# arpg/vicalib

Hardware: AMD Instinct MI355X
Metric: corner_residuals_per_sec (higher is better)
Workload: dtype f64

## Files before the change

vicalib_amd/csrc/vc_imu.hpp:

```cpp
#pragma once
#include "vc_math.hpp"

namespace vc {

struct D1 { double a, v; };
VC_HD D1 mk(double a, double v = 0.0) { D1 r; r.a = a; r.v = v; return r; }
VC_HD D1 operator+(D1 x, D1 y) { return mk(x.a + y.a, x.v + y.v); }
VC_HD D1 operator-(D1 x, D1 y) { return mk(x.a - y.a, x.v - y.v); }
VC_HD D1 operator-(D1 x) { return mk(-x.a, -x.v); }
VC_HD D1 operator*(D1 x, D1 y) { return mk(x.a * y.a, x.a * y.v + x.v * y.a); }
VC_HD D1 operator/(D1 x, D1 y) { const double inv = fast_rcp(y.a), q = x.a * inv; return mk(q, (x.v - q * y.v) * inv); }
VC_HD D1 operator+(D1 x, double s) { return mk(x.a + s, x.v); }
VC_HD D1 operator+(double s, D1 x) { return mk(x.a + s, x.v); }
VC_HD D1 operator-(D1 x, double s) { return mk(x.a - s, x.v); }
VC_HD D1 operator-(double s, D1 x) { return mk(s - x.a, -x.v); }
VC_HD D1 operator*(D1 x, double s) { return mk(x.a * s, x.v * s); }
VC_HD D1 operator*(double s, D1 x) { return mk(x.a * s, x.v * s); }
VC_HD D1 operator/(D1 x, double s) { const double inv = 1.0 / s; return mk(x.a * inv, x.v * inv); }
VC_HD D1 operator/(double s, D1 y) { const double inv = fast_rcp(y.a); return mk(s * inv, -s * inv * inv * y.v); }
VC_HD bool operator<(D1 x, double y) { return x.a < y; }
VC_HD bool operator>(D1 x, double y) { return x.a > y; }
VC_HD D1 sqrt(D1 x) { double s, is; fast_sqrt_rsqrt(x.a, &s, &is); return mk(s, 0.5 * x.v * is); }
VC_HD D1 sin(D1 x) { return mk(::sin(x.a), ::cos(x.a) * x.v); }
VC_HD D1 cos(D1 x) { return mk(::cos(x.a), -::sin(x.a) * x.v); }
// ... 304 lines not shown
  J[0 * 6 + 3] = 0.5 * q0; J[0 * 6 + 4] = -0.5 * q3; J[0 * 6 + 5] = 0.5 * q2;
  J[1 * 6 + 3] = 0.5 * q3; J[1 * 6 + 4] = 0.5 * q0; J[1 * 6 + 5] = -0.5 * q1;
  J[2 * 6 + 3] = -0.5 * q2; J[2 * 6 + 4] = 0.5 * q1; J[2 * 6 + 5] = 0.5 * q0;
  J[3 * 6 + 3] = -0.5 * q1; J[3 * 6 + 4] = -0.5 * q2; J[3 * 6 + 5] = -0.5 * q3;
  J[4 * 6 + 0] = 1.0 - 2.0 * (q2 * q2 + q3 * q3); J[4 * 6 + 1] = 2.0 * (q1 * q2 - q0 * q3); J[4 * 6 + 2] = 2.0 * (q1 * q3 + q0 * q2);
  J[5 * 6 + 0] = 2.0 * (q1 * q2 + q0 * q3); J[5 * 6 + 1] = 1.0 - 2.0 * (q1 * q1 + q3 * q3); J[5 * 6 + 2] = 2.0 * (q2 * q3 - q0 * q1);
  J[6 * 6 + 0] = 2.0 * (q1 * q3 - q0 * q2); J[6 * 6 + 1] = 2.0 * (q2 * q3 + q0 * q1); J[6 * 6 + 2] = 1.0 - 2.0 * (q1 * q1 + q2 * q2);
}

VC_HD void imu_block_direction(const ImuView& buf, double t_start, double t_end, const double* w_sqrt, int rotation_only,
                               const double* T2, const double* T1, const double* v2, const double* v1, const double* gdir,
                               const double* b, const double* sf, double toff, int dir, double* r, double* dr) {
  D1 P[35];
  for (int i = 0; i < 7; ++i) { P[i] = mk(T2[i]); P[7 + i] = mk(T1[i]); }
  for (int i = 0; i < 3; ++i) { P[14 + i] = mk(v2[i]); P[17 + i] = mk(v1[i]); }
  P[20] = mk(gdir[0]); P[21] = mk(gdir[1]);
  for (int i = 0; i < 6; ++i) { P[22 + i] = mk(b[i]); P[28 + i] = mk(sf[i]); }
  P[34] = mk(toff);
  for (int i = 0; i < 35; ++i) P[i].v = (i == dir) ? 1.0 : 0.0;
  D1 res[9];
  imu_residual<D1>(buf, t_start, t_end, w_sqrt, rotation_only, P, P + 7, P + 14, P + 17, P + 20, P + 22, P + 28, P[34], res);
  for (int i = 0; i < 9; ++i) { r[i] = res[i].a; dr[i] = res[i].v; }
}

constexpr int kDeltaCols = 14;

template <class T> struct DeltaAcc { T q[4], p[3], v[3], t; };
template <class T> VC_HD void imu_delta_append(DeltaAcc<T>* A, const PoseV<T>& d, T dt) {
  T rp[3], rv[3], q[4];
  tq_rotate(A->q, d.p, rp);
  tq_rotate(A->q, d.v, rv);
  tq_mul(A->q, d.q, q);
  for (int i = 0; i < 3; ++i) {
    A->p[i] = (A->p[i] + A->v[i] * dt) + rp[i];
    A->v[i] = A->v[i] + rv[i];
  }
  for (int i = 0; i < 4; ++i) A->q[i] = q[i];
  A->t = A->t + dt;
}
template <class T> VC_HD void imu_delta_then(DeltaAcc<T>* a, const DeltaAcc<T>& x) {
  PoseV<T> d;
  for (int k = 0; k < 4; ++k) d.q[k] = x.q[k];
  for (int k = 0; k < 3; ++k) { d.p[k] = x.p[k]; d.v[k] = x.v[k]; }
  imu_delta_append(a, d, x.t);
}
template <class T> VC_HD void imu_delta_identity(DeltaAcc<T>* a) {
  for (int k = 0; k < 3; ++k) { a->q[k] = cst<T>(0.0); a->p[k] = cst<T>(0.0); a->v[k] = cst<T>(0.0); }
  a->q[3] = cst<T>(1.0); a->t = cst<T>(0.0);
}
constexpr int kBlockDeltaStride = kDeltaCols * 11;

VC_HD void so3_exp_jl(const double* w, double* q, double* A, double* B) {
  const double th2 = w[0] * w[0] + w[1] * w[1] + w[2] * w[2];
  double imag, real;
  tso3_exp_factors(th2, &imag, &real);
  q[0] = imag * w[0]; q[1] = imag * w[1]; q[2] = imag * w[2]; q[3] = real;
  const bool tiny = th2 < 1e-6;
  *A = 2.0 * imag * imag;
  *B = tiny ? 1.0 / 6.0 - th2 * (1.0 / 120.0) : (1.0 - 2.0 * imag * real) * fast_rcp(tiny ? 1.0 : th2);
}
VC_HD void cross3(const double* a, const double* b, double* o) {
  const double x = a[1] * b[2] - a[2] * b[1], y = a[2] * b[0] - a[0] * b[2], z = a[0] * b[1] - a[1] * b[0];
  o[0] = x; o[1] = y; o[2] = z;
}
VC_HD void so3_jl_apply(const double* w, double A, double B, const double* d, double* o) {
  double c1[3], c2[3];
  cross3(w, d, c1);
  cross3(w, c1, c2);
  for (int i = 0; i < 3; ++i) o[i] = d[i] + A * c1[i] + B * c2[i];
}
VC_HD void mat3_vec(const double* R, const double* v, double* o) {
  const double a = R[0] * v[0] + R[1] * v[1] + R[2] * v[2];
  const double b = R[3] * v[0] + R[4] * v[1] + R[5] * v[2];
  const double c = R[6] * v[0] + R[7] * v[1] + R[8] * v[2];
  o[0] = a; o[1] = b; o[2] = c;
}
struct IntervalDeltaT { DeltaAcc<double> d; double dth[3], dp[3], dv[3], dt; double ap[3], av[3]; };
constexpr int kDtDoubles = 27;
VC_HD void imu_delta_t_identity(IntervalDeltaT* X) {
  imu_delta_identity(&X->d);
  for (int i = 0; i < 3; ++i) { X->dth[i] = 0.0; X->dp[i] = 0.0; X->dv[i] = 0.0; X->ap[i] = 0.0; X->av[i] = 0.0; }
  X->dt = 0.0;
}
VC_HD void imu_interval_delta_t(const ImuView& buf, const ImuRange& rg, D1 off, double t_start, double t_end, int m, int n_int,
                                const double* b, const double* sf, int gsel, IntervalDeltaT* X) {
  imu_delta_t_identity(X);
  const int kk = gsel < 3 ? gsel : (gsel < 6 ? gsel - 3 : 0);
  const bool seeded = gsel < 6, scale = gsel >= 3;
  double u0[3], u1[3], a0[3], a1[3], du0[3], du1[3], da0[3], da1[3], h, dh;
  double c0, c1;
  {
    Meas<D1> z0, z1;
    for (int k = 0; k < 3; ++k) { z0.w[k] = z0.a[k] = z1.w[k] = z1.a[k] = mk(0.0); }
    z0.time = z1.time = mk(0.0);
    if (m <= n_int) { imu_range_get_flat(buf, rg, off, t_start, t_end, m - 1, &z0); imu_range_get_flat(buf, rg, off, t_start, t_end, m, &z1); }
    if (z1.time.a == z0.time.a) return;
    h = z1.time.a - z0.time.a; dh = z1.time.v - z0.time.v;
    for (int i = 0; i < 3; ++i) {
      const double s0 = (seeded && i == kk) ? (scale ? z0.w[i].a : 1.0) : 0.0, s1 = (seeded && i == kk) ? (scale ? z1.w[i].a : 1.0) : 0.0;
      u0[i] = z0.w[i].a * sf[i] + b[i]; du0[i] = z0.w[i].v * sf[i] + s0;
      u1[i] = z1.w[i].a * sf[i] + b[i]; du1[i] = z1.w[i].v * sf[i] + s1;
      a0[i] = z0.a[i].a * sf[3 + i] + b[3 + i]; da0[i] = z0.a[i].v * sf[3 + i];
      a1[i] = z1.a[i].a * sf[3 + i] + b[3 + i]; da1[i] = z1.a[i].v * sf[3 + i];
    }
    c0 = scale ? (kk == 0 ? z0.a[0].a : kk == 1 ? z0.a[1].a : z0.a[2].a) : 1.0;
    c1 = scale ? (kk == 0 ? z1.a[0].a : kk == 1 ? z1.a[1].a : z1.a[2].a) : 1.0;
  }
  const double hh = h * 0.5, h6 = h / 6.0, dhh = dh * 0.5, dh6 = dh / 6.0;
  const double cm = 0.5 * c0 + 0.5 * c1;
  double sw[3], sv[3], sp[3], dsw[3], dsv[3], dsp[3], cv[3], cp[3], phi[3], dphi[3];
  for (int i = 0; i < 3; ++i) {
    sw[i] = u0[i]; dsw[i] = du0[i]; sv[i] = a0[i]; dsv[i] = da0[i]; sp[i] = a0[i]; dsp[i] = da0[i];
    cv[i] = (i == kk) ? c0 : 0.0; cp[i] = cv[i];
    phi[i] = u0[i] * hh; dphi[i] = du0[i] * hh + u0[i] * dhh;
  }
  for (int stage = 2; stage <= 4; ++stage) {
    double q[4], A, B, R[9], dth[3], ug[3], ua[3], dug[3], dua[3], wk[3], ak[3], dwk[3], dak[3], t1[3], t2[3];
    so3_exp_jl(phi, q, &A, &B);
    quat_to_R(q, R);
    so3_jl_apply(phi, A, B, dphi, dth);
    for (int i = 0; i < 3; ++i) {
      if (stage < 4) { ug[i] = u0[i] * 0.5 + u1[i] * 0.5; ua[i] = a0[i] * 0.5 + a1[i] * 0.5; dug[i] = du0[i] * 0.5 + du1[i] * 0.5; dua[i] = da0[i] * 0.5 + da1[i] * 0.5; }
      else { ug[i] = u1[i]; ua[i] = a1[i]; dug[i] = du1[i]; dua[i] = da1[i]; }
    }
    mat3_vec(R, ug, wk); mat3_vec(R, ua, ak);
    cross3(dth, wk, t1); mat3_vec(R, dug, t2);
    for (int i = 0; i < 3; ++i) dwk[i] = t1[i] + t2[i];
    cross3(dth, ak, t1); mat3_vec(R, dua, t2);
    for (int i = 0; i < 3; ++i) dak[i] = t1[i] + t2[i];
    const double r[3] = {kk == 0 ? R[0] : kk == 1 ? R[1] : R[2], kk == 0 ? R[3] : kk == 1 ? R[4] : R[5], kk == 0 ? R[6] : kk == 1 ? R[7] : R[8]};
    const double wgt = stage < 4 ? 2.0 : 1.0, cc = stage < 4 ? cm : c1;
    for (int i = 0; i < 3; ++i) {
      sw[i] = sw[i] + wgt * wk[i]; dsw[i] = dsw[i] + wgt * dwk[i];
      sv[i] = sv[i] + wgt * ak[i]; dsv[i] = dsv[i] + wgt * dak[i];
      cv[i] = cv[i] + wgt * (cc * r[i]);
      if (stage < 4) { sp[i] = sp[i] + ak[i]; dsp[i] = dsp[i] + dak[i]; cp[i] = cp[i] + cc * r[i]; }
      const double hs = stage == 2 ? hh : h, dhs = stage == 2 ? dhh : dh;
      if (stage < 4) { phi[i] = wk[i] * hs; dphi[i] = dwk[i] * hs + wk[i] * dhs; }
    }
  }
  {
    double A, B;
    for (int i = 0; i < 3; ++i) { phi[i] = sw[i] * h6; dphi[i] = dsw[i] * h6 + sw[i] * dh6; }
    so3_exp_jl(phi, X->d.q, &A, &B);
    so3_jl_apply(phi, A, B, dphi, X->dth);
    const double hh6 = h * h6, dhh6 = 2.0 * h * dh6;
    for (int i = 0; i < 3; ++i) {
      X->d.v[i] = sv[i] * h6; X->dv[i] = dsv[i] * h6 + sv[i] * dh6;
      X->d.p[i] = sp[i] * hh6; X->dp[i] = dsp[i] * hh6 + sp[i] * dhh6;
      X->av[i] = cv[i] * h6; X->ap[i] = cp[i] * hh6;
    }
    X->d.t = h; X->dt = dh;
  }
}
VC_HD void imu_delta_t_then(IntervalDeltaT* A, const IntervalDeltaT& X) {
  double R[9], rp[3], rv[3], t1[3], t2[3], t3[3], q[4];
  quat_to_R(A->d.q, R);
  mat3_vec(R, X.d.p, rp); mat3_vec(R, X.d.v, rv);
  cross3(A->dth, rp, t1); mat3_vec(R, X.dp, t2);
  for (int i = 0; i < 3; ++i) A->dp[i] = ((A->dp[i] + A->dv[i] * X.d.t) + A->d.v[i] * X.dt) + (t1[i] + t2[i]);
  cross3(A->dth, rv, t1); mat3_vec(R, X.dv, t2);
  for (int i = 0; i < 3; ++i) A->dv[i] = A->dv[i] + (t1[i] + t2[i]);
  mat3_vec(R, X.dth, t3);
  for (int i = 0; i < 3; ++i) A->dth[i] = A->dth[i] + t3[i];
  A->dt = A->dt + X.dt;
  mat3_vec(R, X.ap, t1); mat3_vec(R, X.av, t2);
  for (int i = 0; i < 3; ++i) {
    A->ap[i] = (A->ap[i] + A->av[i] * X.d.t) + t1[i];
    A->av[i] = A->av[i] + t2[i];
  }
  for (int i = 0; i < 3; ++i) {
    A->d.p[i] = (A->d.p[i] + A->d.v[i] * X.d.t) + rp[i];
    A->d.v[i] = A->d.v[i] + rv[i];
  }
  quat_mul(A->d.q, X.d.q, q);
  for (int i = 0; i < 4; ++i) A->d.q[i] = q[i];
  A->d.t = A->d.t + X.d.t;
}
VC_HD int imu_group_dual_col(int g) { return g < 3 ? 1 + g : (g < 6 ? 4 + g : 13); }
VC_HD int imu_group_accel_col(int g) { return g < 3 ? 4 + g : 7 + g; }
VC_HD void imu_block_record_store(const IntervalDeltaT& X, int g, double* rec) {
  if (g > 6) return;
  double* cd = rec + imu_group_dual_col(g) * 11;
  const double hq[4] = {0.5 * X.dth[0], 0.5 * X.dth[1], 0.5 * X.dth[2], 0.0};
  double dq[4];
  quat_mul(hq, X.d.q, dq);
  for (int k = 0; k < 4; ++k) cd[k] = dq[k];
  for (int k = 0; k < 3; ++k) { cd[4 + k] = X.dp[k]; cd[7 + k] = X.dv[k]; }
  cd[10] = X.dt;
  if (g < 6) {
    double* ca = rec + imu_group_accel_col(g) * 11;
    for (int k = 0; k < 4; ++k) ca[k] = 0.0;
    for (int k = 0; k < 3; ++k) { ca[4 + k] = X.ap[k]; ca[7 + k] = X.av[k]; }
    ca[10] = 0.0;
  }
  if (g == 0) {
    for (int k = 0; k < 4; ++k) rec[k] = X.d.q[k];
    for (int k = 0; k < 3; ++k) { rec[4 + k] = X.d.p[k]; rec[7 + k] = X.d.v[k]; }
    rec[10] = X.d.t;
  }
}
inline int imu_block_delta_record(const ImuView& buf, double t_start, double t_end, double toff, const double* b, const double* sf,
                                  double* rec ) {
  const ImuRange rg = imu_range(buf, t_start, t_end, toff);
  if (!rg.valid) { rec[10] = -1.0; return 0; }
  const int n_int = (rg.k1 - rg.k0 + 1) + 1;
  for (int g = 0; g < 7; ++g) {
    const D1 offD = mk(toff, g == 6 ? 1.0 : 0.0);
    IntervalDeltaT carry;
    for (int base = 0; base < n_int; base += 16) {
      IntervalDeltaT X[8], Y[8];
      for (int l = 0; l < 8; ++l) {
        IntervalDeltaT second;
        imu_interval_delta_t(buf, rg, offD, t_start, t_end, base + 2 * l + 1, n_int, b, sf, g, &X[l]);
        imu_interval_delta_t(buf, rg, offD, t_start, t_end, base + 2 * l + 2, n_int, b, sf, g, &second);
        imu_delta_t_then(&X[l], second);
      }
      for (int n = 1; n < 8; n <<= 1) {
        for (int l = 0; l < 8; ++l) { Y[l] = X[l]; if (l >= n) { Y[l] = X[l - n]; imu_delta_t_then(&Y[l], X[l]); } }
        for (int l = 0; l < 8; ++l) X[l] = Y[l];
      }
      if (base == 0) carry = X[7]; else imu_delta_t_then(&carry, X[7]);
    }
    imu_block_record_store(carry, g, rec);
  }
  return 1;
}

VC_HD void imu_block_final_direction(int valid, const double* block_rec, const double* w_sqrt, int rotation_only, const double* T2,
                                     const double* T1, const double* v2, const double* v1, const double* grav9 , int col,
                                     double* r, double* dr) {
  if (!valid) { for (int i = 0; i < 9; ++i) { r[i] = 0.0; dr[i] = 0.0; } return; }
  const int dcol = (col >= 20) ? col - 19 : 0;
  D1 Q[4], P[3], V[3];
  double bd[11];
  for (int k = 0; k < 11; ++k) { const double d = block_rec[dcol * 11 + k]; bd[k] = dcol ? d : 0.0; }
  for (int k = 0; k < 4; ++k) Q[k] = mk(block_rec[k], bd[k]);
  for (int k = 0; k < 3; ++k) { P[k] = mk(block_rec[4 + k], bd[4 + k]); V[k] = mk(block_rec[7 + k], bd[7 + k]); }
  const D1 Tt = mk(block_rec[10], bd[10]);
  D1 T2D[7], v2D[3], gw[3], q0[4], p0[3], v0[3];
  {
    double J[42];
    local_jac_se3(T2, J);
    for (int i = 0; i < 7; ++i) {
      double sel = 0.0;
      for (int c = 0; c < 6; ++c) sel = (col == c) ? J[i * 6 + c] : sel;
      T2D[i] = mk(T2[i], sel);
    }
    local_jac_se3(T1, J);
    for (int i = 0; i < 7; ++i) {
      double sel = 0.0;
      for (int c = 0; c < 6; ++c) sel = (col == 9 + c) ? J[i * 6 + c] : sel;
      if (i < 4) q0[i] = mk(T1[i], sel); else p0[i - 4] = mk(T1[i], sel);
    }
  }
  for (int k = 0; k < 3; ++k) { v2D[k] = mk(v2[k], col == 6 + k ? 1.0 : 0.0); v0[k] = mk(v1[k], col == 15 + k ? 1.0 : 0.0); }
  for (int k = 0; k < 3; ++k) gw[k] = mk(grav9[k], col == 18 ? grav9[3 + k] : (col == 19 ? grav9[6 + k] : 0.0));
  PoseV<D1> x;
  D1 rp[3], rv[3];
  tq_rotate(q0, P, rp);
  tq_rotate(q0, V, rv);
  tq_mul(q0, Q, x.q);
  const D1 ht2 = 0.5 * (Tt * Tt);
  for (int i = 0; i < 3; ++i) {
    x.p[i] = ((p0[i] + v0[i] * Tt) - gw[i] * ht2) + rp[i];
    x.v[i] = (v0[i] - gw[i] * Tt) + rv[i];
  }
  D1 res[9];
  imu_residual_tail(x, w_sqrt, rotation_only, T2D, v2D, res);
  for (int i = 0; i < 9; ++i) { r[i] = res[i].a; dr[i] = res[i].v; }
}

}
```

vicalib_amd/csrc/vc_imu_kernels.hip:

```cpp
#include <hip/hip_runtime.h>
#include <algorithm>
#include <cstdlib>
#include "vc_math.hpp"
#include "vc_imu.hpp"
#include "vc_imu_weights.hpp"
#include "vc_device.h"
#include "vc_kutil.hpp"
#include "vc_reduced_tail.hpp"
#include "vc_shared_blocks.hpp"

namespace vc {

__device__ __forceinline__ ImuView imu_view(const DevView& v) { ImuView b = {v.imu_t, v.imu_w, v.imu_a, v.n_imu, v.imu_avg_dt}; return b; }

constexpr int kImuJacLds = 34 * 9 + 6;
struct SegTab {
  unsigned short v[kSegStride];
  constexpr SegTab() : v() { for (int e = 0; e < kSegLen; ++e) { int a = 0, b = 0; seg_entry(e, &a, &b); v[e] = (unsigned short)(a | (b << 8)); } }
};
__constant__ SegTab d_seg_tab = SegTab();
constexpr int kSegIters = (kSegLen + 31) / 32;
#ifndef VC_IJ_MFMA
#define VC_IJ_MFMA 1
#endif
// ... 183 lines not shown
  for (int e = 0; e < N; ++e) x[e] += y[e];
}
template <int N> __device__ __forceinline__ void row_allsum_n(double* x) {
  row_add_level<0xB1, N>(x);
  row_add_level<0x4E, N>(x);
  row_add_level<0x141, N>(x);
  row_add_level<0x140, N>(x);
}
__device__ __forceinline__ double shfl16(double x, int src) { return __shfl(x, src, 16); }
__device__ __forceinline__ void delta_identity(DeltaAcc<double>* a) {
#pragma unroll
  for (int k = 0; k < 3; ++k) { a->q[k] = 0.0; a->p[k] = 0.0; a->v[k] = 0.0; }
  a->q[3] = 1.0; a->t = 0.0;
}
__device__ __forceinline__ void delta_then(DeltaAcc<double>* a, const DeltaAcc<double>& x) {
  PoseV<double> d;
#pragma unroll
  for (int k = 0; k < 4; ++k) d.q[k] = x.q[k];
#pragma unroll
  for (int k = 0; k < 3; ++k) { d.p[k] = x.p[k]; d.v[k] = x.v[k]; }
  imu_delta_append(a, d, x.t);
}
template <int N> __device__ __forceinline__ void delta_scan_level(DeltaAcc<double>* X, int c) {
  DeltaAcc<double> A;
#pragma unroll
  for (int k = 0; k < 4; ++k) A.q[k] = row_shr<N>(X->q[k], X->q[k]);
#pragma unroll
  for (int k = 0; k < 3; ++k) { A.p[k] = row_shr<N>(X->p[k], X->p[k]); A.v[k] = row_shr<N>(X->v[k], X->v[k]); }
  A.t = row_shr<N>(X->t, X->t);
  delta_then(&A, *X);
  if (c >= N) *X = A;
}
template <int N> __device__ __forceinline__ void map_scan_level(double* S) {
  double B[kWMapF], O[kWMapF];
  w_map_identity(B);
#pragma unroll
  for (int e = 0; e < kWMapF; ++e) B[e] = row_shl<N>(B[e], S[e]);
  w_map_compose(B, S, O);
#pragma unroll
  for (int e = 0; e < kWMapF; ++e) S[e] = O[e];
}

__device__ __forceinline__ ImuRange imu_range_lanes(const ImuView& b, double t0, double t1, double off, int lane) {
  ImuRange r; r.valid = 0; r.k0 = 0; r.k1 = -1; r.i0 = r.i1 = 0; r.first_end = r.last_end = 0;
  if (b.n < 2) return r;
  const bool odd = lane & 1;
  int idx, endc, le;
  imu_element_index(b, odd ? t1 : t0, off, &idx, &endc, &le);
  const int idx_o = __shfl_xor(idx, 1, 64), endc_o = __shfl_xor(endc, 1, 64), le_o = __shfl_xor(le, 1, 64);
  r.valid = (t0 >= b.t[0] + off && t0 <= b.t[b.n - 1] + off) ? 1 : 0;
  r.i0 = odd ? idx_o : idx; r.first_end = odd ? endc_o : endc;
  r.i1 = odd ? idx : idx_o; r.last_end = odd ? endc : endc_o;
  r.k0 = r.i0 + 1;
  r.k1 = odd ? le : le_o;
  if (r.k1 < r.i0) r.k1 = r.i0;
  return r;
}

__device__ __forceinline__ void delta_t_pack(const IntervalDeltaT& X, double* f) {
#pragma unroll
  for (int k = 0; k < 4; ++k) f[k] = X.d.q[k];
#pragma unroll
  for (int k = 0; k < 3; ++k) { f[4 + k] = X.d.p[k]; f[7 + k] = X.d.v[k]; f[11 + k] = X.dth[k]; f[14 + k] = X.dp[k]; f[17 + k] = X.dv[k]; f[21 + k] = X.ap[k]; f[24 + k] = X.av[k]; }
  f[10] = X.d.t; f[20] = X.dt;
}
__device__ __forceinline__ void delta_t_unpack(const double* f, IntervalDeltaT* X) {
#pragma unroll
  for (int k = 0; k < 4; ++k) X->d.q[k] = f[k];
#pragma unroll
  for (int k = 0; k < 3; ++k) { X->d.p[k] = f[4 + k]; X->d.v[k] = f[7 + k]; X->dth[k] = f[11 + k]; X->dp[k] = f[14 + k]; X->dv[k] = f[17 + k]; X->ap[k] = f[21 + k]; X->av[k] = f[24 + k]; }
  X->d.t = f[10]; X->dt = f[20];
}
template <int N> __device__ __forceinline__ void delta_t_scan_level(IntervalDeltaT* X, int l) {
  double f[kDtDoubles];
  delta_t_pack(*X, f);
#pragma unroll
  for (int k = 0; k < kDtDoubles; ++k) f[k] = row_shr<N>(f[k], f[k]);
  IntervalDeltaT A;
  delta_t_unpack(f, &A);
  imu_delta_t_then(&A, *X);
  if (l >= N) *X = A;
}
#ifdef VC_IB_STAMPS
#define IBSTAMP(i) do { if (blockIdx.x == gridDim.x / 2 && threadIdx.x == 0) v.dbg[i] = (long long)__builtin_amdgcn_s_memrealtime(); } while (0)
#else
#define IBSTAMP(i) do { } while (0)
#endif
#ifndef VC_IMU_BLOCK_WAVES
#define VC_IMU_BLOCK_WAVES 2
#endif
#ifdef VC_IMU_BLOCK_EU
__global__ __launch_bounds__(256) __attribute__((amdgpu_waves_per_eu(VC_IMU_BLOCK_EU, VC_IMU_BLOCK_EU))) void k_imu_block(DevView v, int trial) {
#else
__global__ __launch_bounds__(256, VC_IMU_BLOCK_WAVES) void k_imu_block(DevView v, int trial) {
#endif
  __shared__ double s_carry[32 * kDtDoubles];
  __shared__ double s_park[256 * (kDtDoubles - 11)];
  __shared__ double s_parkv[4 * 8 * 11];
  IBSTAMP(0);
  if (trial && v.sync_seq > 0 && workgroup_pass_void(v)) return;
  const int lane = threadIdx.x & 63, wave = __builtin_amdgcn_readfirstlane(threadIdx.x >> 6);
  const int g = lane >> 3, l = lane & 7;
  const int n_blocks = v.n_frames - 1;
  const int s_raw = blockIdx.x * 4 + wave;
  const int s = s_raw < n_blocks ? s_raw : n_blocks - 1;
  const double toff0 = v.imus[0][14], toff1 = v.imus[1][14];
  const double t_start = v.frame_time[s], t_end = v.frame_time[s + 1];
  const Ctrl* ct = v.ctrl;
  const int c_done = ct->done, c_need = ct->need_lin, c_cur = ct->cur;
  if (c_done || (!trial && !c_need)) return;
  IBSTAMP(1);
  const int cur = trial ? 1 - c_cur : c_cur;
  const double* im = v.imus[cur];
  const double toff = cur ? toff1 : toff0;
  const ImuView buf = imu_view(v);
  ImuRange rg = imu_range_lanes(buf, t_start, t_end, toff, lane);
  rg.valid = __builtin_amdgcn_readfirstlane(rg.valid); rg.i0 = __builtin_amdgcn_readfirstlane(rg.i0); rg.i1 = __builtin_amdgcn_readfirstlane(rg.i1);
  rg.k0 = __builtin_amdgcn_readfirstlane(rg.k0); rg.k1 = __builtin_amdgcn_readfirstlane(rg.k1);
  rg.first_end = __builtin_amdgcn_readfirstlane(rg.first_end); rg.last_end = __builtin_amdgcn_readfirstlane(rg.last_end);
  double* rec = v.imu_delta_blk + (size_t)s * kBlockDeltaStride;
  IBSTAMP(2);
  if (rg.valid) {
    const int n_int = (rg.k1 - rg.k0 + 1) + 1;
    const int gsel = g < 7 ? g : 6;
    double* cr = s_carry + (threadIdx.x >> 3) * kDtDoubles;
    IntervalDeltaT X;
#pragma unroll 1
    for (int base = 0; base < n_int; base += 16) {
      {
        IntervalDeltaT Y;
        double* pk = s_park + threadIdx.x;
        double* pv = s_parkv + (wave * 8 + l) * 11;
#pragma unroll 1
        for (int half = 0; half < 2; ++half) {
          int gs = gsel;
          asm volatile("" : "+v"(gs));
          imu_interval_delta_t(buf, rg, mk(toff, gs == 6 ? 1.0 : 0.0), t_start, t_end, base + 2 * l + 1 + half, n_int, im + 2, im + 8, gs, &Y);
          IBSTAMP(3 + half);
          if (half == 0) {
            double f[kDtDoubles];
            delta_t_pack(Y, f);
#pragma unroll
            for (int k = 11; k < kDtDoubles; ++k) pk[(k - 11) * 256] = f[k];
            if (g == 0) {
#pragma unroll
              for (int k = 0; k < 11; ++k) pv[k] = f[k];
            }
          }
        }
        wave_lds_sync_local();
        double f[kDtDoubles];
#pragma unroll
        for (int k = 0; k < 11; ++k) f[k] = pv[k];
#pragma unroll
        for (int k = 11; k < kDtDoubles; ++k) f[k] = pk[(k - 11) * 256];
        delta_t_unpack(f, &X);
        wave_lds_sync_local();
        imu_delta_t_then(&X, Y);
      }
      IBSTAMP(5);
      delta_t_scan_level<1>(&X, l); delta_t_scan_level<2>(&X, l); delta_t_scan_level<4>(&X, l);
      IBSTAMP(6);
      if (l == 7) {
        if (base > 0) {
          IntervalDeltaT A;
          double f[kDtDoubles];
#pragma unroll
          for (int k = 0; k < kDtDoubles; ++k) f[k] = cr[k];
          delta_t_unpack(f, &A);
          imu_delta_t_then(&A, X);
          X = A;
        }
        if (base + 16 < n_int) {
          double f[kDtDoubles];
          delta_t_pack(X, f);
#pragma unroll
          for (int k = 0; k < kDtDoubles; ++k) cr[k] = f[k];
        }
      }
    }
    if (l == 7 && s_raw < n_blocks) imu_block_record_store(X, g, rec);
    IBSTAMP(7);
  } else if (lane == 0 && s_raw < n_blocks) rec[10] = -1.0;
  if (blockIdx.x == 0 && threadIdx.x == 63) imu_gravity_record(im, v.imu_grav + cur * 16);
  if (trial && v.block_wait > 0 && blockIdx.x == 0 && threadIdx.x == 0) spin_until_flag<false>(v, 2, v.block_wait);
}

#ifdef VC_W_STAMPS
#define WSTAMP(i) do { if (blockIdx.x == 0 && threadIdx.x == 0) v.dbg[i] = (long long)__builtin_amdgcn_s_memrealtime(); } while (0)
#else
#define WSTAMP(i) do { } while (0)
#endif
__global__ __launch_bounds__(64) void k_imu_weights(DevView v, int wr) {
  __shared__ __attribute__((aligned(16))) double w_lds[4 * kWLds];
  const Ctrl* ct = v.ctrl;
  const int lane = threadIdx.x;
  const int grp = lane >> 4, c = lane & 15;
  const int n_blocks = v.n_frames - 1;
  const int s_raw = blockIdx.x * 4 + grp;
  const bool exists = s_raw < n_blocks;
  const int s = exists ? s_raw : n_blocks - 1;
  double* L = w_lds + grp * kWLds;
  if (v.sync_seq > 0) { const long long m = sync_marked(v); if (m != 0 && m <= v.sync_seq) return; }
  if (ct->done == kDoneSyncTimeout) return;
  if (ct->done || !v.weights_on) {
    if (exists) for (int e = c; e < 81; e += 16) v.wsqrtb[1 - wr][(size_t)s * 81 + e] = v.wsqrtb[wr][(size_t)s * 81 + e];
    return;
  }
  WSTAMP(0);
  const int j = s + 1;
  {
    const double p0 = v.poses[0][(size_t)(j - 1) * kPoseStride + c], p1 = v.poses[1][(size_t)(j - 1) * kPoseStride + c];
    const double u0 = v.vel[0][(size_t)(j - 1) * 4 + (c & 3)], u1 = v.vel[1][(size_t)(j - 1) * 4 + (c & 3)];
    const int ci = c < 15 ? c : 14;
    const double i0 = v.imus[0][ci], i1 = v.imus[1][ci];
    const bool one = ct->cur != 0;
    L[kWPose + c] = one ? p1 : p0;
    if (c < 4) L[kWVel + c] = one ? u1 : u0;
    if (c < 15) L[kWImu + c] = one ? i1 : i0;
  }
  const double t_start = v.frame_time[j - 1], t_end = v.frame_time[j];
  wave_lds_sync();
  double b[6], sf[6];
#pragma unroll
  for (int i = 0; i < 6; ++i) { b[i] = L[kWImu + 2 + i]; sf[i] = L[kWImu + 8 + i]; }
  const double toff = L[kWImu + 14];
  const ImuView buf = imu_view(v);
  const ImuRange rg = imu_range_lanes(buf, t_start, t_end, toff, lane);
  const bool live = exists && rg.valid;
  const double sg2 = v.gyro_sigma * v.gyro_sigma, sa2 = v.accel_sigma * v.accel_sigma;
  const int n_int = live ? (rg.k1 - rg.k0 + 1) + 1 : 0;
  int n_max = n_int;
#pragma unroll
  for (int o = 32; o >= 16; o >>= 1) n_max = max(n_max, __shfl_xor(n_max, o, 64));
  DeltaAcc<double> carry;
  delta_identity(&carry);
  const double g0[3] = {0.0, 0.0, 0.0};
  WSTAMP(1);
#pragma unroll 1
  for (int base = 0; base < n_max; base += 16) {
    const int m = base + c + 1;
    Meas<double> z0, z1;
#pragma unroll
    for (int k = 0; k < 3; ++k) { z0.w[k] = z0.a[k] = z1.w[k] = z1.a[k] = 0.0; }
    z0.time = z1.time = 0.0;
    if (m <= n_int) { imu_range_get_flat(buf, rg, toff, t_start, t_end, m - 1, &z0); imu_range_get_flat(buf, rg, toff, t_start, t_end, m, &z1); }
    const bool act = z1.time != z0.time;
    WSTAMP(2);
    DeltaAcc<double> X;
    {
      PoseV<double> d;
#pragma unroll
      for (int k = 0; k < 3; ++k) { d.q[k] = 0.0; d.p[k] = 0.0; d.v[k] = 0.0; }
      d.q[3] = 1.0;
      imu_rk4_step(&d, z0, z1, b, sf, g0);
#pragma unroll
      for (int k = 0; k < 4; ++k) X.q[k] = d.q[k];
#pragma unroll
      for (int k = 0; k < 3; ++k) { X.p[k] = d.p[k]; X.v[k] = d.v[k]; }
      X.t = z1.time - z0.time;
    }
    WSTAMP(3);
    delta_scan_level<1>(&X, c); delta_scan_level<2>(&X, c); delta_scan_level<4>(&X, c); delta_scan_level<8>(&X, c);
    double q_st[4];
    {
      double qe[4], ident[4] = {0.0, 0.0, 0.0, 1.0};
// ... 2169 lines not shown
#pragma unroll
      for (int u = 0; u < NL; ++u) {
        const unsigned qf = (unsigned)(row * 57) >> 9;
        const bool masked = (mbits >> qf) & 1u;
        tmp[u] = (row < nrow && !masked) ? src[(unsigned)(row * v.ldx + col) + qf * skip] : 0.0;
        row += step_r; col += step_c;
        if (col >= ld) { col -= ld; ++row; }
      }
    };
    request(f0);
    for (int fg = f0; fg < f1; fg += 4) {
#pragma unroll
      for (int u = 0; u < NL; ++u) { const int i = tid + 256 * u; if (i < 36 * ld) R[i] = tmp[u]; }
      __syncthreads();
      GSTAMP(gs_); ++gs_;
      if (fg + 4 < f1) request(fg + 4);
      const double* rq = R + (lane >> 4) * ld + (lane & 15);
      int oa[NQ], ob[NQ];
#pragma unroll
      for (int q = 0; q < NQ; ++q) {
        const int p = min(pb + 4 * q + wave, nPairs - 1);
        const int ij = s_pair[p];
        oa[q] = (ij & 255) * 16; ob[q] = (ij >> 8) * 16;
      }
#pragma unroll
      for (int ks = 0; ks < 9; ++ks)
#pragma unroll
        for (int q = 0; q < NQ; ++q) acc[q] = __builtin_amdgcn_mfma_f64_16x16x4f64(rq[ks * 4 * ld + oa[q]], rq[ks * 4 * ld + ob[q]], acc[q], 0, 0, 0);
      __syncthreads();
      GSTAMP(gs_); ++gs_;
    }
#pragma unroll
    for (int q = 0; q < NQ; ++q) {
      const int p = pb + 4 * q + wave;
      if (p < nPairs) {
        const int ij = s_pair[p], I = ij & 255, J = ij >> 8;
#pragma unroll
        for (int g = 0; g < 4; ++g) {
          const int row = I * 16 + (lane >> 4) + 4 * g, col = J * 16 + (lane & 15);
          if (row < D && col <= D) {
            double* dst = col < D ? part + row * D + col : part + D * D + row;
            if (publish) __hip_atomic_store(dst, acc[q][g], __ATOMIC_RELAXED, __HIP_MEMORY_SCOPE_AGENT); else *dst = acc[q][g];
          }
        }
      }
    }
  }
  if (publish) {
    __builtin_amdgcn_s_waitcnt(0);
    __syncthreads();
    if (tid == 0) __hip_atomic_store(v.part_ready + chunk, v.pass_id, __ATOMIC_RELAXED, __HIP_MEMORY_SCOPE_AGENT);
  }
#ifdef VC_GRAM_STAMPS
  __builtin_amdgcn_s_waitcnt(0);
  GSTAMP(15);
#endif
}
template <int NQ, int NL>
__global__ __launch_bounds__(256, 2) void k_chain_gram(DevView v, int gather) {
  extern __shared__ __attribute__((aligned(16))) double R[];
  __shared__ unsigned short s_pair[128];
  if (gather) chain_gram_chunk<NQ, NL>(v, v.n_chunks, R, s_pair, 0, v.gram_top_stride);
  else chain_gram_chunk<NQ, NL>(v, (int)blockIdx.x, R, s_pair, v.gram_top_stride);
}
template <int NW, int NQ, int NL>
__global__ __launch_bounds__(256) void k_chain_top_gram(DevView v, int s, int m, int lvl) {
  extern __shared__ __attribute__((aligned(16))) double R[];
  __shared__ unsigned short s_pair[128];
  __shared__ __attribute__((aligned(16))) double XS[9 * kXsLd];
  __shared__ double An[81];
  __shared__ double Ls_all[NW * 81];
  if (blockIdx.x == 0) {
    if ((int)threadIdx.x >= 64 * NW) return;
    chain_fwd_group<1, NW>(v, s, m, 1, lvl, 0, (int)(threadIdx.x >> 6), XS, An, Ls_all);
    return;
  }
  if ((int)blockIdx.x == 1 + v.n_chunks) { hadd_side_job(v, R, 256); return; }
  if ((int)blockIdx.x > 1 + v.n_chunks) { part_sum_ride_job(v, (int)blockIdx.x - 2 - v.n_chunks, R); return; }
  chain_gram_chunk<NQ, NL>(v, (int)blockIdx.x - 1, R, s_pair, v.gram_top_stride, 0, v.part_ride != 0);
}

void launch_imu_delta(const DevView& v, hipStream_t s, int trial) {
  if (v.n_frames < 2) return;
  hipLaunchKernelGGL(k_imu_block, dim3((v.n_frames - 1 + 3) / 4), dim3(256), 0, s, v, trial);
}
void launch_imu_jac(const DevView& v, int wr, hipStream_t s, int trial) {
  if (v.n_frames < 2) return;
  hipLaunchKernelGGL(k_imu_jac, dim3((v.n_frames - 1 + 7) / 8), dim3(256), 0, s, v, wr, trial);
}
void launch_imu_weights(const DevView& v, int wr, hipStream_t s) {
  if (v.n_frames < 2) return;
  hipLaunchKernelGGL(k_imu_weights, dim3((v.n_frames - 1 + 3) / 4), dim3(64), 0, s, v, wr);
}
void launch_chain_gram(const DevView& v, hipStream_t s);
static void chain_levels(const DevView& v, const ChainPlan& p, hipStream_t s, bool forward) {
  const int N = v.n_frames;
  if (N < 1) return;
  const int nl = p.n_levels, top_stride = p.top_stride, m_top = kChainM;
  const int cpl = (v.D + 1 + 27 + 63) / 64;
  auto fwd = [&](int groups, int stride, int m, int top, int lvl) {
    if (!top && p.two[lvl]) {
      const int extra = (v.hadd_early && lvl == 1) ? (v.part_stride - (v.D * v.D + v.D) + 15) / 16 : 0;
      if (cpl <= 1) hipLaunchKernelGGL(k_chain_fwd2<1>, dim3(groups + extra), dim3(128), 0, s, v, stride, m, lvl, groups);
      else hipLaunchKernelGGL(k_chain_fwd2<2>, dim3(groups + extra), dim3(256), 0, s, v, stride, m, lvl, groups);
    }
    else if (cpl <= 1) hipLaunchKernelGGL((k_chain_fwd<1, 1>), dim3(groups), dim3(64), 0, s, v, stride, m, top, lvl);
    else if (cpl <= 2) hipLaunchKernelGGL((k_chain_fwd<1, 2>), dim3(groups), dim3(128), 0, s, v, stride, m, top, lvl);
    else if (cpl <= 3) hipLaunchKernelGGL((k_chain_fwd<1, 3>), dim3(groups), dim3(192), 0, s, v, stride, m, top, lvl);
    else hipLaunchKernelGGL((k_chain_fwd<1, 4>), dim3(groups), dim3(256), 0, s, v, stride, m, top, lvl);
  };
  if (forward) {
    for (int l = 0; l < nl; ++l) {
      if (l == 0 && v.fold_l0) {
        if (v.n_cams <= 1) hipLaunchKernelGGL(k_chain_l0<1>, dim3(p.groups[0]), dim3(256), 0, s, v);
        else hipLaunchKernelGGL(k_chain_l0<2>, dim3(p.groups[0]), dim3(256), 0, s, v);
      } else fwd(p.groups[l], p.stride[l], p.m[l], 0, l);
    }
    if (v.gram_top_stride > 0) {
      const size_t lds = std::max((size_t)36 * v.ldw, (size_t)(v.hadd_early ? kHaddLds : 0)) * sizeof(double);
      const int ride_blocks = (v.part_ride && v.hadd_early) ? (v.D * v.D + v.D + 15) / 16 : 0;
      const int nT = (v.D + 1 + 15) / 16, nPairs = nT * (nT + 1) / 2, nq = std::min(kMaxPairsPerWaveI, (nPairs + 3) / 4);
      const int nlr = (36 * v.ldw + 255) / 256;
      auto go = [&](auto kern) {
        if (lds > 40000) (void)hipFuncSetAttribute((const void*)kern, hipFuncAttributeMaxDynamicSharedMemorySize, (int)lds);
        hipLaunchKernelGGL(kern, dim3(1 + v.n_chunks + (v.hadd_early ? 1 : 0) + ride_blocks), dim3(256), lds, s, v, top_stride, m_top, nl);
      };
      if (cpl <= 1) { if (nq <= 1) go(k_chain_top_gram<1, 1, 7>); else go(k_chain_top_gram<1, 2, 7>); }
      else if (cpl <= 2) { if (nlr <= 12) go(k_chain_top_gram<2, 4, 12>); else if (nq <= 6) go(k_chain_top_gram<2, 6, 16>); else go(k_chain_top_gram<2, 9, 16>); }
      else if (cpl <= 3) { if (nlr <= 16) go(k_chain_top_gram<3, 9, 16>); else if (nlr <= 21) go(k_chain_top_gram<3, 9, 21>); else go(k_chain_top_gram<3, 9, 25>); }
      else { if (nlr <= 25) go(k_chain_top_gram<4, 9, 25>); else go(k_chain_top_gram<4, 9, 30>); }
    } else {
      fwd(1, top_stride, m_top, 1, nl);
    }
  } else {
    if (v.back_path && nl >= 1 && nl <= 5) {
      BackPath P; P.n = nl;
      for (int l = 0; l < 6; ++l) { P.stride[l] = l < nl ? p.stride[l] : 1; P.m[l] = l < nl ? p.m[l] : 2; P.two[l] = l < nl ? p.two[l] : 0; }
      const bool ct0 = v.D + 1 > kPathRowCols;
      P.top_stride = top_stride; P.ldr = ct0 ? 1 : ((v.D + 1) | 1); P.dsw = ((v.D + 63) / 64) * 64;
      if (ct0) hipLaunchKernelGGL(k_chain_t0, dim3((N + 3) / 4), dim3(256), 0, s, v);
      const int nw = nl + 1;
      P.tail = (v.tail_deferred && nw >= 4) ? 1 : 0;
      const size_t lds = std::max(((size_t)nw * kPathDl + (size_t)nw * P.dsw + 4 + (ct0 ? 0 : (size_t)nw * 63 * P.ldr)), (size_t)(P.tail ? kTailLds : 0)) * sizeof(double);
      static LdsGrant g4, g6;
      auto go = [&](auto kern, LdsGrant& g) {
        if (lds > 60000 && g.need(lds)) (void)hipFuncSetAttribute((const void*)kern, hipFuncAttributeMaxDynamicSharedMemorySize, (int)lds);
        hipLaunchKernelGGL(kern, dim3(p.groups[0] + P.tail), dim3(64 * nw), lds, s, v, P);
      };
      if (nw <= 4) { if (ct0) go(k_chain_back_path<4, true>, g4); else go(k_chain_back_path<4, false>, g4); }
      else { if (ct0) go(k_chain_back_path<6, true>, g6); else go(k_chain_back_path<6, false>, g6); }
      return;
    }
    hipLaunchKernelGGL(k_chain_back, dim3(1 + (nl > 0 ? (N + kBackT0Frames - 1) / kBackT0Frames : 0)), dim3(64), 0, s, v, top_stride, m_top, 1, nl, 0);
    int total_groups = 0;
    for (int l = 0; l < nl; ++l) total_groups += p.groups[l];
    static const int resident_limit = [] {
      int dev = 0, per_cu = 0; hipDeviceProp_t pr;
      if (hipGetDevice(&dev) != hipSuccess || hipGetDeviceProperties(&pr, dev) != hipSuccess ||
          hipOccupancyMaxActiveBlocksPerMultiprocessor(&per_cu, (const void*)k_chain_back_levels, 64, 0) != hipSuccess || per_cu <= 0) return 2048;
      return std::max(64, per_cu * pr.multiProcessorCount / 2);
    }();
    if (nl > 0 && nl <= 8 && v.cready && total_groups <= resident_limit) {
      BackLevels L; L.n = nl;
      int at = 0;
      for (int i = 0; i < nl; ++i) {
        const int l = nl - 1 - i;
        L.start[i] = at; L.stride[i] = p.stride[l]; L.m[i] = p.m[l]; L.two[i] = p.two[l];
// ... 40 lines not shown
```

Measured before the change: 2.124 billion.

## Process IMU block deltas with four sequential intervals per lane, two blocks per wave

The IMU block kernel changes its work split. Each lane now integrates a run of four consecutive intervals serially, with a 4-lane scan instead of 8, and each wave handles two frame blocks (half-waves), so the grid shrinks by half. Adjacent interval endpoints are passed through LDS instead of being re-interpolated, which avoids redundant element fetches. Interval evaluation is refactored into an element-based core shared with the host reference path. The trade-off is longer serial chains per lane and extra LDS syncs, in exchange for fewer scan levels and better lane utilisation.

```diff
diff --git a/vicalib_amd/csrc/vc_imu.hpp b/vicalib_amd/csrc/vc_imu.hpp
--- a/vicalib_amd/csrc/vc_imu.hpp
+++ b/vicalib_amd/csrc/vc_imu.hpp
@@ -410,18 +410,13 @@
   for (int i = 0; i < 3; ++i) { X->dth[i] = 0.0; X->dp[i] = 0.0; X->dv[i] = 0.0; X->ap[i] = 0.0; X->av[i] = 0.0; }
   X->dt = 0.0;
 }
-VC_HD void imu_interval_delta_t(const ImuView& buf, const ImuRange& rg, D1 off, double t_start, double t_end, int m, int n_int,
-                                const double* b, const double* sf, int gsel, IntervalDeltaT* X) {
+VC_HD void imu_elements_delta_t(const Meas<D1>& z0, const Meas<D1>& z1, const double* b, const double* sf, int gsel, IntervalDeltaT* X) {
   imu_delta_t_identity(X);
   const int kk = gsel < 3 ? gsel : (gsel < 6 ? gsel - 3 : 0);
   const bool seeded = gsel < 6, scale = gsel >= 3;
   double u0[3], u1[3], a0[3], a1[3], du0[3], du1[3], da0[3], da1[3], h, dh;
   double c0, c1;
   {
-    Meas<D1> z0, z1;
-    for (int k = 0; k < 3; ++k) { z0.w[k] = z0.a[k] = z1.w[k] = z1.a[k] = mk(0.0); }
-    z0.time = z1.time = mk(0.0);
-    if (m <= n_int) { imu_range_get_flat(buf, rg, off, t_start, t_end, m - 1, &z0); imu_range_get_flat(buf, rg, off, t_start, t_end, m, &z1); }
     if (z1.time.a == z0.time.a) return;
     h = z1.time.a - z0.time.a; dh = z1.time.v - z0.time.v;
     for (int i = 0; i < 3; ++i) {
@@ -434,7 +429,7 @@
     c0 = scale ? (kk == 0 ? z0.a[0].a : kk == 1 ? z0.a[1].a : z0.a[2].a) : 1.0;
     c1 = scale ? (kk == 0 ? z1.a[0].a : kk == 1 ? z1.a[1].a : z1.a[2].a) : 1.0;
   }
-  const double hh = h * 0.5, h6 = h / 6.0, dhh = dh * 0.5, dh6 = dh / 6.0;
+  const double hh = h * 0.5, dhh = dh * 0.5;
   const double cm = 0.5 * c0 + 0.5 * c1;
   double sw[3], sv[3], sp[3], dsw[3], dsv[3], dsp[3], cv[3], cp[3], phi[3], dphi[3];
   for (int i = 0; i < 3; ++i) {
@@ -442,6 +437,9 @@
     cv[i] = (i == kk) ? c0 : 0.0; cp[i] = cv[i];
     phi[i] = u0[i] * hh; dphi[i] = du0[i] * hh + u0[i] * dhh;
   }
+#if defined(__HIP_DEVICE_COMPILE__)
+#pragma unroll 1
+#endif
   for (int stage = 2; stage <= 4; ++stage) {
     double q[4], A, B, R[9], dth[3], ug[3], ua[3], dug[3], dua[3], wk[3], ak[3], dwk[3], dak[3], t1[3], t2[3];
     so3_exp_jl(phi, q, &A, &B);
@@ -468,6 +466,7 @@
     }
   }
   {
+    const double h6 = h / 6.0, dh6 = dh / 6.0;
     double A, B;
     for (int i = 0; i < 3; ++i) { phi[i] = sw[i] * h6; dphi[i] = dsw[i] * h6 + sw[i] * dh6; }
     so3_exp_jl(phi, X->d.q, &A, &B);
@@ -480,6 +479,14 @@
     }
     X->d.t = h; X->dt = dh;
   }
+}
+VC_HD void imu_interval_delta_t(const ImuView& buf, const ImuRange& rg, D1 off, double t_start, double t_end, int m, int n_int,
+                                const double* b, const double* sf, int gsel, IntervalDeltaT* X) {
+  Meas<D1> z0, z1;
+  for (int k = 0; k < 3; ++k) { z0.w[k] = z0.a[k] = z1.w[k] = z1.a[k] = mk(0.0); }
+  z0.time = z1.time = mk(0.0);
+  if (m <= n_int) { imu_range_get_flat(buf, rg, off, t_start, t_end, m - 1, &z0); imu_range_get_flat(buf, rg, off, t_start, t_end, m, &z1); }
+  imu_elements_delta_t(z0, z1, b, sf, gsel, X);
 }
 VC_HD void imu_delta_t_then(IntervalDeltaT* A, const IntervalDeltaT& X) {
   double R[9], rp[3], rv[3], t1[3], t2[3], t3[3], q[4];
@@ -505,6 +512,85 @@
   for (int i = 0; i < 4; ++i) A->d.q[i] = q[i];
   A->d.t = A->d.t + X.d.t;
 }
+VC_HD void imu_range_element_t(const ImuView& b, const ImuRange& r, double off, bool tdir, double t0, double t1, int which, Meas<D1>* m) {
+  const int n_int = r.k1 - r.k0 + 1;
+  const bool first = which == 0, last = which > n_int;
+  const int idx = first ? r.i0 : (last ? r.i1 : r.k0 + which - 1);
+  const bool interp = (first && !r.first_end) || (last && !r.last_end);
+  const int idn = idx + 1 < b.n ? idx + 1 : b.n - 1;
+  const double tq = first ? t0 : t1;
+  const double ta_ = b.t[idx], tb_ = b.t[idn];
+  double wa[3], wb[3], aa[3], ab[3];
+  for (int k = 0; k < 3; ++k) { wa[k] = b.w[3 * idx + k]; wb[k] = b.w[3 * idn + k]; aa[k] = b.a[3 * idx + k]; ab[k] = b.a[3 * idn + k]; }
+  const double ta = ta_ + off, tb = tb_ + off;
+  const double den = interp ? tb - ta : 1.0;
+  const double inv = fast_rcp(den);
+  const double f = (tq - ta) * inv;
+  const double omf = 1.0 - f;
+  const double df = (interp && tdir) ? -inv : 0.0;
+  for (int k = 0; k < 3; ++k) {
+    const double wi = wa[k] * omf + wb[k] * f, ai = aa[k] * omf + ab[k] * f;
+    m->w[k] = mk(interp ? wi : wa[k], (wb[k] - wa[k]) * df);
+    m->a[k] = mk(interp ? ai : aa[k], (ab[k] - aa[k]) * df);
+  }
+  m->time = mk(interp ? tq : ta, (!interp && tdir) ? 1.0 : 0.0);
+}
+constexpr int kImuRunLen = 4;
+struct ImuBlockCtx { ImuRange rg; double t_start, t_end; int n_int; };
+template <class Park>
+VC_HD void imu_run_delta_t(const ImuView& buf, double toff, int base, const double* b, const double* sf, Park& park, IntervalDeltaT* X) {
+#if defined(__HIP_DEVICE_COMPILE__)
+#pragma unroll 1
+#endif
+  for (int j = 0; j < kImuRunLen; ++j) {
+    const int gs = park.direction();
+    const bool tdir = gs == 6;
+    const int m = base + kImuRunLen * park.lane() + 1 + j;
+    Meas<D1> z0, z1;
+    for (int k = 0; k < 3; ++k) { z0.w[k] = z0.a[k] = z1.w[k] = z1.a[k] = mk(0.0); }
+    z0.time = z1.time = mk(0.0);
+    {
+      ImuBlockCtx cx;
+      park.block(&cx);
+      if (m <= cx.n_int) {
+        if (j == 0) imu_range_element_t(buf, cx.rg, toff, tdir, cx.t_start, cx.t_end, m - 1, &z0);
+        else {
+          double e[7];
+          park.elem_load(e);
+          for (int k = 0; k < 3; ++k) { z0.w[k] = mk(e[k]); z0.a[k] = mk(e[3 + k]); }
+          z0.time = mk(e[6], tdir ? 1.0 : 0.0);
+        }
+        imu_range_element_t(buf, cx.rg, toff, tdir, cx.t_start, cx.t_end, m, &z1);
+        if (j + 1 < kImuRunLen) {
+          const double e[7] = {z1.w[0].a, z1.w[1].a, z1.w[2].a, z1.a[0].a, z1.a[1].a, z1.a[2].a, z1.time.a};
+          park.elem_store(e);
+        }
+      }
+    }
+    IntervalDeltaT Y;
+    imu_elements_delta_t(z0, z1, b, sf, gs, &Y);
+    if (j == 0) park.store(Y);
+    else {
+      IntervalDeltaT A;
+      park.load(&A);
+      imu_delta_t_then(&A, Y);
+      park.store(A);
+    }
+    park.step_done(j);
+  }
+  park.load(X);
+}
+struct HostPark {
+  ImuBlockCtx cx; IntervalDeltaT s; double e[7]; int l, g;
+  int lane() const { return l; }
+  int direction() const { return g; }
+  void block(ImuBlockCtx* c) const { *c = cx; }
+  void elem_store(const double* x) { for (int k = 0; k < 7; ++k) e[k] = x[k]; }
+  void elem_load(double* x) const { for (int k = 0; k < 7; ++k) x[k] = e[k]; }
+  void store(const IntervalDeltaT& x) { s = x; }
+  void load(IntervalDeltaT* x) const { *x = s; }
+  void step_done(int) const {}
+};
 VC_HD int imu_group_dual_col(int g) { return g < 3 ? 1 + g : (g < 6 ? 4 + g : 13); }
 VC_HD int imu_group_accel_col(int g) { return g < 3 ? 4 + g : 7 + g; }
 VC_HD void imu_block_record_store(const IntervalDeltaT& X, int g, double* rec) {
@@ -529,26 +615,27 @@
   }
 }
 inline int imu_block_delta_record(const ImuView& buf, double t_start, double t_end, double toff, const double* b, const double* sf,
-                                  double* rec ) {
+                                  double* rec , int* n_intervals = nullptr) {
   const ImuRange rg = imu_range(buf, t_start, t_end, toff);
+  if (n_intervals) *n_intervals = 0;
   if (!rg.valid) { rec[10] = -1.0; return 0; }
   const int n_int = (rg.k1 - rg.k0 + 1) + 1;
+  if (n_intervals) *n_intervals = n_int;
+  constexpr int kLanes = 16 / kImuRunLen;
   for (int g = 0; g < 7; ++g) {
-    const D1 offD = mk(toff, g == 6 ? 1.0 : 0.0);
     IntervalDeltaT carry;
     for (int base = 0; base < n_int; base += 16) {
-      IntervalDeltaT X[8], Y[8];
-      for (int l = 0; l < 8; ++l) {
-        IntervalDeltaT second;
-        imu_interval_delta_t(buf, rg, offD, t_start, t_end, base + 2 * l + 1, n_int, b, sf, g, &X[l]);
-        imu_interval_delta_t(buf, rg, offD, t_start, t_end, base + 2 * l + 2, n_int, b, sf, g, &second);
-        imu_delta_t_then(&X[l], second);
+      IntervalDeltaT X[kLanes], Y[kLanes];
+      for (int l = 0; l < kLanes; ++l) {
+        HostPark park;
+        park.cx.rg = rg; park.cx.t_start = t_start; park.cx.t_end = t_end; park.cx.n_int = n_int; park.l = l; park.g = g;
+        imu_run_delta_t(buf, toff, base, b, sf, park, &X[l]);
       }
-      for (int n = 1; n < 8; n <<= 1) {
-        for (int l = 0; l < 8; ++l) { Y[l] = X[l]; if (l >= n) { Y[l] = X[l - n]; imu_delta_t_then(&Y[l], X[l]); } }
-        for (int l = 0; l < 8; ++l) X[l] = Y[l];
+      for (int n = 1; n < kLanes; n <<= 1) {
+        for (int l = 0; l < kLanes; ++l) { Y[l] = X[l]; if (l >= n) { Y[l] = X[l - n]; imu_delta_t_then(&Y[l], X[l]); } }
+        for (int l = 0; l < kLanes; ++l) X[l] = Y[l];
       }
-      if (base == 0) carry = X[7]; else imu_delta_t_then(&carry, X[7]);
+      if (base == 0) carry = X[kLanes - 1]; else imu_delta_t_then(&carry, X[kLanes - 1]);
     }
     imu_block_record_store(carry, g, rec);
   }
diff --git a/vicalib_amd/csrc/vc_imu_kernels.hip b/vicalib_amd/csrc/vc_imu_kernels.hip
--- a/vicalib_amd/csrc/vc_imu_kernels.hip
+++ b/vicalib_amd/csrc/vc_imu_kernels.hip
@@ -289,27 +289,79 @@
   if (l >= N) *X = A;
 }
 #ifdef VC_IB_STAMPS
-#define IBSTAMP(i) do { if (blockIdx.x == gridDim.x / 2 && threadIdx.x == 0) v.dbg[i] = (long long)__builtin_amdgcn_s_memrealtime(); } while (0)
+#define IBSTAMP_AT(dbg, i) do { if (blockIdx.x == gridDim.x / 2 && threadIdx.x == 0) (dbg)[i] = (long long)__builtin_amdgcn_s_memrealtime(); } while (0)
 #else
-#define IBSTAMP(i) do { } while (0)
-#endif
+#define IBSTAMP_AT(dbg, i) do { } while (0)
+#endif
+#define IBSTAMP(i) IBSTAMP_AT(v.dbg, i)
+constexpr int kBlkInts = 8;
+struct BlockRunPark {
+  double* s_park; double* s_parkv; double* s_elem; const int* s_blki; const double* s_blkt; long long* dbg;
+  __device__ __forceinline__ int tid() const { int t = threadIdx.x; asm volatile("" : "+v"(t)); return t; }
+  __device__ __forceinline__ int lane() const { return tid() & 3; }
+  __device__ __forceinline__ int direction() const { const int g = (tid() >> 2) & 7; return g < 7 ? g : 6; }
+  __device__ __forceinline__ void block(ImuBlockCtx* c) const {
+    const int hb = tid() >> 5;
+    const int* i = s_blki + hb * kBlkInts; const double* t = s_blkt + hb * 2;
+    c->rg.valid = 1; c->rg.i0 = i[0]; c->rg.first_end = i[1]; c->rg.k0 = i[2]; c->rg.k1 = i[3]; c->rg.i1 = i[4]; c->rg.last_end = i[5];
+    c->n_int = i[6]; c->t_start = t[0]; c->t_end = t[1];
+  }
+  __device__ __forceinline__ void elem_store(const double* e) const {
+    const int t = tid();
+    if ((t & 28) == 0) {
+      double* pe = s_elem + ((t >> 5) * 4 + (t & 3)) * 7;
+#pragma unroll
+      for (int k = 0; k < 7; ++k) pe[k] = e[k];
+    }
+  }
+  __device__ __forceinline__ void elem_load(double* e) const {
+    const int t = tid();
+    const double* pe = s_elem + ((t >> 5) * 4 + (t & 3)) * 7;
+    wave_lds_sync_local();
+#pragma unroll
+    for (int k = 0; k < 7; ++k) e[k] = pe[k];
+    wave_lds_sync_local();
+  }
+  __device__ __forceinline__ void store(const IntervalDeltaT& Y) const {
+    const int t = tid();
+    double* pk = s_park + t;
+    double f[kDtDoubles];
+    delta_t_pack(Y, f);
+#pragma unroll
+    for (int k = 11; k < kDtDoubles; ++k) pk[(k - 11) * 256] = f[k];
+    if ((t & 28) == 0) {
+      double* pv = s_parkv + ((t >> 5) * 4 + (t & 3)) * 11;
+#pragma unroll
+      for (int k = 0; k < 11; ++k) pv[k] = f[k];
+    }
+  }
+  __device__ __forceinline__ void load(IntervalDeltaT* X) const {
+    const int t = tid();
+    const double* pk = s_park + t;
+    const double* pv = s_parkv + ((t >> 5) * 4 + (t & 3)) * 11;
+    wave_lds_sync_local();
+    double f[kDtDoubles];
+#pragma unroll
+    for (int k = 0; k < 11; ++k) f[k] = pv[k];
+#pragma unroll
+    for (int k = 11; k < kDtDoubles; ++k) f[k] = pk[(k - 11) * 256];
+    delta_t_unpack(f, X);
+    wave_lds_sync_local();
+  }
+  __device__ __forceinline__ void step_done(int j) const { IBSTAMP_AT(dbg, 3 + j); }
+};
 #ifndef VC_IMU_BLOCK_WAVES
 #define VC_IMU_BLOCK_WAVES 2
 #endif
-#ifdef VC_IMU_BLOCK_EU
-__global__ __launch_bounds__(256) __attribute__((amdgpu_waves_per_eu(VC_IMU_BLOCK_EU, VC_IMU_BLOCK_EU))) void k_imu_block(DevView v, int trial) {
-#else
 __global__ __launch_bounds__(256, VC_IMU_BLOCK_WAVES) void k_imu_block(DevView v, int trial) {
-#endif
-  __shared__ double s_carry[32 * kDtDoubles];
+  __shared__ double s_carry[64 * kDtDoubles];
   __shared__ double s_park[256 * (kDtDoubles - 11)];
-  __shared__ double s_parkv[4 * 8 * 11];
+  __shared__ double s_parkv[8 * 4 * 11];
   IBSTAMP(0);
   if (trial && v.sync_seq > 0 && workgroup_pass_void(v)) return;
-  const int lane = threadIdx.x & 63, wave = __builtin_amdgcn_readfirstlane(threadIdx.x >> 6);
-  const int g = lane >> 3, l = lane & 7;
+  const int lane = threadIdx.x & 63;
   const int n_blocks = v.n_frames - 1;
-  const int s_raw = blockIdx.x * 4 + wave;
+  const int s_raw = blockIdx.x * 8 + (threadIdx.x >> 5);
   const int s = s_raw < n_blocks ? s_raw : n_blocks - 1;
   const double toff0 = v.imus[0][14], toff1 = v.imus[1][14];
   const double t_start = v.frame_time[s], t_end = v.frame_time[s + 1];
@@ -317,68 +369,50 @@
   const int c_done = ct->done, c_need = ct->need_lin, c_cur = ct->cur;
   if (c_done || (!trial && !c_need)) return;
   IBSTAMP(1);
-  const int cur = trial ? 1 - c_cur : c_cur;
+  const int cur = __builtin_amdgcn_readfirstlane(trial ? 1 - c_cur : c_cur);
   const double* im = v.imus[cur];
-  const double toff = cur ? toff1 : toff0;
+  const double toff_v = cur ? toff1 : toff0;
+  const double toff = __hiloint2double(__builtin_amdgcn_readfirstlane(__double2hiint(toff_v)), __builtin_amdgcn_readfirstlane(__double2loint(toff_v)));
   const ImuView buf = imu_view(v);
-  ImuRange rg = imu_range_lanes(buf, t_start, t_end, toff, lane);
-  rg.valid = __builtin_amdgcn_readfirstlane(rg.valid); rg.i0 = __builtin_amdgcn_readfirstlane(rg.i0); rg.i1 = __builtin_amdgcn_readfirstlane(rg.i1);
-  rg.k0 = __builtin_amdgcn_readfirstlane(rg.k0); rg.k1 = __builtin_amdgcn_readfirstlane(rg.k1);
-  rg.first_end = __builtin_amdgcn_readfirstlane(rg.first_end); rg.last_end = __builtin_amdgcn_readfirstlane(rg.last_end);
-  double* rec = v.imu_delta_blk + (size_t)s * kBlockDeltaStride;
+  __shared__ int s_blki[8 * kBlkInts];
+  __shared__ double s_blkt[8 * 2];
+  __shared__ double s_elem[8 * 4 * 7];
+  const int hb = threadIdx.x >> 5;
+  int n_max;
+  {
+    const ImuRange rg = imu_range_lanes(buf, t_start, t_end, toff, lane);
+    const int n_int = rg.valid ? (rg.k1 - rg.k0 + 1) + 1 : 0;
+    const int n_other = __shfl_xor(n_int, 32, 64);
+    n_max = __builtin_amdgcn_readfirstlane(n_int > n_other ? n_int : n_other);
+    if ((lane & 31) == 0) {
+      int* i = s_blki + hb * kBlkInts;
+      i[0] = rg.i0; i[1] = rg.first_end; i[2] = rg.k0; i[3] = rg.k1; i[4] = rg.i1; i[5] = rg.last_end; i[6] = n_int;
+      s_blkt[hb * 2] = t_start; s_blkt[hb * 2 + 1] = t_end;
+    }
+    wave_lds_sync_local();
+  }
   IBSTAMP(2);
-  if (rg.valid) {
-    const int n_int = (rg.k1 - rg.k0 + 1) + 1;
-    const int gsel = g < 7 ? g : 6;
-    double* cr = s_carry + (threadIdx.x >> 3) * kDtDoubles;
+  {
+    BlockRunPark park = {s_park, s_parkv, s_elem, s_blki, s_blkt, v.dbg};
     IntervalDeltaT X;
 #pragma unroll 1
-    for (int base = 0; base < n_int; base += 16) {
-      {
-        IntervalDeltaT Y;
-        double* pk = s_park + threadIdx.x;
-        double* pv = s_parkv + (wave * 8 + l) * 11;
-#pragma unroll 1
-        for (int half = 0; half < 2; ++half) {
-          int gs = gsel;
-          asm volatile("" : "+v"(gs));
-          imu_interval_delta_t(buf, rg, mk(toff, gs == 6 ? 1.0 : 0.0), t_start, t_end, base + 2 * l + 1 + half, n_int, im + 2, im + 8, gs, &Y);
-          IBSTAMP(3 + half);
-          if (half == 0) {
-            double f[kDtDoubles];
-            delta_t_pack(Y, f);
-#pragma unroll
-            for (int k = 11; k < kDtDoubles; ++k) pk[(k - 11) * 256] = f[k];
-            if (g == 0) {
-#pragma unroll
-              for (int k = 0; k < 11; ++k) pv[k] = f[k];
-            }
-          }
-        }
-        wave_lds_sync_local();
-        double f[kDtDoubles];
-#pragma unroll
-        for (int k = 0; k < 11; ++k) f[k] = pv[k];
-#pragma unroll
-        for (int k = 11; k < kDtDoubles; ++k) f[k] = pk[(k - 11) * 256];
-        delta_t_unpack(f, &X);
-        wave_lds_sync_local();
-        imu_delta_t_then(&X, Y);
-      }
-      IBSTAMP(5);
-      delta_t_scan_level<1>(&X, l); delta_t_scan_level<2>(&X, l); delta_t_scan_level<4>(&X, l);
-      IBSTAMP(6);
-      if (l == 7) {
+    for (int base = 0; base < n_max; base += 16) {
+      imu_run_delta_t(buf, toff, base, im + 2, im + 8, park, &X);
+      const int t = park.tid(), l = t & 3;
+      delta_t_scan_level<1>(&X, l); delta_t_scan_level<2>(&X, l);
+      IBSTAMP(7);
+      if (l == 3) {
+        double* cr = s_carry + (t >> 2) * kDtDoubles;
         if (base > 0) {
           IntervalDeltaT A;
           double f[kDtDoubles];
 #pragma unroll
           for (int k = 0; k < kDtDoubles; ++k) f[k] = cr[k];
           delta_t_unpack(f, &A);
-          imu_delta_t_then(&A, X);
+          if (base < s_blki[(t >> 5) * kBlkInts + 6]) imu_delta_t_then(&A, X);
           X = A;
         }
-        if (base + 16 < n_int) {
+        if (base + 16 < n_max) {
           double f[kDtDoubles];
           delta_t_pack(X, f);
 #pragma unroll
@@ -386,9 +420,14 @@
         }
       }
     }
-    if (l == 7 && s_raw < n_blocks) imu_block_record_store(X, g, rec);
-    IBSTAMP(7);
-  } else if (lane == 0 && s_raw < n_blocks) rec[10] = -1.0;
+    const int t = park.tid(), sr = blockIdx.x * 8 + (t >> 5);
+    if (sr < n_blocks) {
+      double* rec = v.imu_delta_blk + (size_t)sr * kBlockDeltaStride;
+      if (s_blki[(t >> 5) * kBlkInts + 6] > 0) { if ((t & 3) == 3) imu_block_record_store(X, (t >> 2) & 7, rec); }
+      else if ((t & 31) == 0) rec[10] = -1.0;
+    }
+    IBSTAMP(8);
+  }
   if (blockIdx.x == 0 && threadIdx.x == 63) imu_gravity_record(im, v.imu_grav + cur * 16);
   if (trial && v.block_wait > 0 && blockIdx.x == 0 && threadIdx.x == 0) spin_until_flag<false>(v, 2, v.block_wait);
 }
@@ -2724,7 +2763,7 @@
 
 void launch_imu_delta(const DevView& v, hipStream_t s, int trial) {
   if (v.n_frames < 2) return;
-  hipLaunchKernelGGL(k_imu_block, dim3((v.n_frames - 1 + 3) / 4), dim3(256), 0, s, v, trial);
+  hipLaunchKernelGGL(k_imu_block, dim3((v.n_frames - 1 + 7) / 8), dim3(256), 0, s, v, trial);
 }
 void launch_imu_jac(const DevView& v, int wr, hipStream_t s, int trial) {
   if (v.n_frames < 2) return;
```

Result: slower. 2.078 billion (-2.1%).
